# mrottmann/DDalphaAMG

Hardware: AMD Instinct MI355X
Metric: fine_wilson_clover_gflops (higher is better)
Workload: dtype f32; 1 GPU; fine Wilson-Clover apply (d_plus_clover), 32x32x32x32 local lattice per GPU, random SU(3) gauge, csw=1.0, anti-periodic T; parallelism=single, ranks=1

## Files before the change

### ddalphaamg_amd/api.py

```python
import ctypes, os, re
import numpy as np

_HERE = os.path.dirname(os.path.abspath(__file__))
_LIBNAME = os.environ.get("DDAMG_HIP_LIBRARY") or os.path.join(_HERE, "libddamg_hip.so")
_HEADER = os.path.join(os.path.dirname(_HERE), "include", "ddamg_hip.h")
MAX_LEVELS = 4
MAX_FORCE_PAIRS = 32
FORCE_GROUP = 8


class DDAMGError(RuntimeError):
    pass


class Params(ctypes.Structure):
    _fields_ = [
        ("num_levels", ctypes.c_int),
        ("local_lattice", (ctypes.c_int * 4) * MAX_LEVELS),
        ("block_lattice", (ctypes.c_int * 4) * MAX_LEVELS),
        ("num_vect", ctypes.c_int * MAX_LEVELS),
        ("post_smooth_iter", ctypes.c_int * MAX_LEVELS),
        ("block_iter", ctypes.c_int * MAX_LEVELS),
        ("setup_iter", ctypes.c_int * MAX_LEVELS),
        ("restart", ctypes.c_int), ("max_restart", ctypes.c_int),
# ... 157 lines not shown
        "ddamg_hip_force_bilinear_multi_vec": [vp, dp, ctypes.c_int, ctypes.POINTER(vp), ctypes.POINTER(vp), dp, ctypes.c_double, ctypes.c_int],
        "ddamg_hip_force_bilinear_multi_device": [vp, dp, ctypes.c_int, ctypes.POINTER(dp), ctypes.POINTER(dp), dp, ctypes.c_double, ctypes.c_int],
        "ddamg_hip_force_bilinear_multi_vec_grid": [vp, dp, ctypes.c_int, ctypes.POINTER(vp), ctypes.POINTER(vp), dp, ctypes.c_double, ctypes.c_int],
        "ddamg_hip_force_bilinear_multi_device_grid": [vp, dp, ctypes.c_int, ctypes.POINTER(dp), ctypes.POINTER(dp), dp, ctypes.c_double, ctypes.c_int],
        "ddamg_hip_force_rational_device": [vp, dp, ctypes.c_int, dp, ctypes.POINTER(dp), ctypes.POINTER(dp), ctypes.c_double, ctypes.c_int],
        "ddamg_hip_force_rational_device_grid": [vp, dp, ctypes.c_int, dp, ctypes.POINTER(dp), ctypes.POINTER(dp), ctypes.c_double, ctypes.c_int],
        "ddamg_hip_preconditioner": [vp, dp, dp],
        "ddamg_hip_residual_history": [vp, dp, ctypes.c_int, ctypes.POINTER(ctypes.c_int)],
        "ddamg_hip_get_site_order": [vp, ctypes.c_int, ctypes.POINTER(ctypes.c_int)],
        "ddamg_hip_rccl_unique_id": [vp],
        "ddamg_hip_comm_init_rccl": [vp, vp],
        "ddamg_hip_comm_init_host": [vp, EXCHANGE_FN, ALLREDUCE_FN, vp],
        "ddamg_hip_halo_plan": [ctypes.POINTER(ctypes.c_int)] * 3 + [ctypes.c_int] + [ctypes.POINTER(ctypes.c_int)] * 3,
        "ddamg_hip_timer_begin": [vp],
        "ddamg_hip_timer_end": [vp, ctypes.POINTER(ctypes.c_float)],
        "ddamg_hip_sync": [vp],
        "ddamg_hip_link_reals": [vp, ctypes.POINTER(ctypes.c_int)],
        "ddamg_hip_memory_in_use": [ctypes.POINTER(ctypes.c_size_t), ctypes.POINTER(ctypes.c_size_t)],
    }
    for name, args in sigs.items():
        fn = getattr(lib, name)
        fn.argtypes = args
        fn.restype = ctypes.c_int
    _lib = lib
    return lib


def memory_in_use():
    dev = ctypes.c_size_t(0); pin = ctypes.c_size_t(0)
    load_library().ddamg_hip_memory_in_use(ctypes.byref(dev), ctypes.byref(pin))
    return dev.value, pin.value


class VectorHeader(ctypes.Structure):
    _fields_ = [("vector_type", ctypes.c_char_p), ("m0", ctypes.c_double), ("csw", ctypes.c_double), ("clov_plaq", ctypes.c_double),
                ("hopp_plaq", ctypes.c_double), ("clov_conf_name", ctypes.c_char_p), ("hopp_conf_name", ctypes.c_char_p),
                ("has_eigenvalues", ctypes.c_int), ("eigenvalues", ctypes.POINTER(ctypes.c_double))]


class LimeInfo(ctypes.Structure):
    _fields_ = [("kind", ctypes.c_int), ("precision", ctypes.c_int), ("lattice", ctypes.c_int * 4), ("has_plaquette", ctypes.c_int),
                ("plaquette", ctypes.c_double), ("data_offset", ctypes.c_longlong), ("data_length", ctypes.c_longlong),
                ("num_records", ctypes.c_int)]


def _io():
    lib = load_library()
    if not getattr(lib, "_io_ready", False):
# ... 330 lines not shown
        cl = np.ascontiguousarray(clover_lex, dtype=np.float64)
        V = self.volume(0)
        if D.size != V * 72 or cl.size != V * 84:
            raise DDAMGError("set_operator: D must be [V][36] complex and clover [V][42] complex")
        _check(self._lib.ddamg_hip_set_operator(self._h, _dp(D), _dp(cl)))

    def shift_mass(self, m0):
        _check(self._lib.ddamg_hip_shift_mass(self._h, float(m0)))

    def scale_clover(self, scale_even, scale_odd):
        _check(self._lib.ddamg_hip_scale_clover(self._h, float(scale_even), float(scale_odd)))

    def get_operator(self):
        V = self.volume(0)
        D = np.empty((V, 36, 2)); cl = np.empty((V, 42, 2))
        _check(self._lib.ddamg_hip_get_operator(self._h, _dp(D), _dp(cl)))
        return D, cl

    def link_reals(self):
        n = ctypes.c_int(0)
        _check(self._lib.ddamg_hip_link_reals(self._h, ctypes.byref(n)))
        return n.value

    def vector(self, level=0, precision=32):
        return Vector(self, level, precision)

    def dirac_apply(self, out, inp):
        _check(self._lib.ddamg_hip_dirac_apply(self._h, out._h, inp._h))

    def dirac_apply_dagger(self, out, inp):
        _check(self._lib.ddamg_hip_dirac_apply_dagger(self._h, out._h, inp._h))

    def gamma5(self, out, inp):
        _check(self._lib.ddamg_hip_gamma5(self._h, out._h, inp._h))

    def vec_copy(self, dst, src):
        _check(self._lib.ddamg_hip_vec_copy(self._h, dst._h, src._h))

    def vec_axpy(self, z, x, y, alpha):
        alpha = complex(alpha)
        _check(self._lib.ddamg_hip_vec_axpy(self._h, z._h, x._h, y._h, alpha.real, alpha.imag))

    def vec_dot(self, x, y):
        re = ctypes.c_double(0); im = ctypes.c_double(0); nx = ctypes.c_double(0)
        _check(self._lib.ddamg_hip_vec_dot(self._h, x._h, y._h, ctypes.byref(re), ctypes.byref(im), ctypes.byref(nx)))
        return complex(re.value, im.value), nx.value
# ... 465 lines not shown
```

### ddalphaamg_amd/csrc/capi.cpp

```cpp
#include "capi_common.h"
#include "gauge.h"
#include "storage_refusal.h"
#include "ildg_device.h"
#include "io_common.h"
#include <algorithm>
#include <cmath>
#include <cstring>
#include <functional>
#include <string>
#include <fcntl.h>

using namespace ddamg;

thread_local std::string g_ddamg_last_error;

ddamg_hip_ctx::~ddamg_hip_ctx() {
  (void)hipSetDevice(device);
  if (stream) (void)hipStreamSynchronize(stream);
  mg32.reset(); mg64.reset();
  if (comm) comm_destroy(comm);
}

double* ddamg_hip_ctx::stage(size_t bytes) {
  if (bytes > d_stage.bytes()) d_stage.alloc(bytes / sizeof(double));
// ... 128 lines not shown
  *out = c.release();
  DDAMG_API_END
}

int ddamg_hip_destroy(ddamg_hip_ctx* c) {
  DDAMG_API_BEGIN
  delete c;
  DDAMG_API_END
}

int ddamg_hip_memory_in_use(size_t* device_bytes, size_t* pinned_bytes) {
  if (device_bytes) *device_bytes = DeviceMemory::in_use.load();
  if (pinned_bytes) *pinned_bytes = PinnedMemory::in_use.load();
  return 0;
}

int ddamg_hip_link_reals(ddamg_hip_ctx* c, int* reals) {
  DDAMG_API_BEGIN
  enter(c);
  DDAMG_REQUIRE(reals, "null argument");
  DDAMG_REQUIRE(c->have_operator, "link_reals: no operator uploaded");
  *reals = c->fop32.link_reals();
  DDAMG_API_END
}

int ddamg_hip_set_coarse_storage(ddamg_hip_ctx* c, int bits) { return set_storage(c, Coarse, bits, "coarse"); }
int ddamg_hip_set_transfer_storage(ddamg_hip_ctx* c, int bits) { return set_storage(c, Transfer, bits, "transfer"); }
int ddamg_hip_set_intermediate_storage(ddamg_hip_ctx* c, int bits) { return set_storage(c, Intermediate, bits, "intermediate"); }

static void drop_clover_base(ddamg_hip_ctx* c) {
  if (c->clover_base) { (void)hipStreamSynchronize(c->stream); c->clover_base.reset(); }
  c->scale_even = c->scale_odd = 1.0;
}

static void rebuild_coarse_operators(ddamg_hip_ctx* c) {
  if (c->setup_done) for_each_mg(c, [](auto& mg) { mg.operator_changed(); mg.release_setup_workspace(); });
}

static void operator_replaced(ddamg_hip_ctx* c) {
  c->have_operator = true;
  rebuild_coarse_operators(c);
}

static void upload_operator(ddamg_hip_ctx* c) {
  drop_clover_base(c);
  const Geometry& g = c->levels[0]->geom;
// ... 916 lines not shown
```

### ddalphaamg_amd/csrc/common.h

```cpp
#pragma once
#include <hip/hip_runtime.h>
#include <cstdio>
#include <cstdlib>
#include <cstdint>
#include <stdexcept>
#include <string>
#include "knobs.h"

#define DDAMG_HIP_CHECK(expr)                                                                  \
  do {                                                                                         \
    hipError_t _e = (expr);                                                                    \
    if (_e != hipSuccess) {                                                                    \
      char _buf[512];                                                                          \
      snprintf(_buf, sizeof _buf, "HIP error %s at %s:%d: %s", hipGetErrorName(_e), __FILE__,  \
               __LINE__, hipGetErrorString(_e));                                               \
      throw std::runtime_error(_buf);                                                          \
    }                                                                                          \
  } while (0)

#define DDAMG_REQUIRE(cond, msg)                                                               \
  do {                                                                                         \
    if (!(cond)) {                                                                             \
      char _buf[512];                                                                          \
      snprintf(_buf, sizeof _buf, "ddamg: requirement failed (%s) at %s:%d: %s", #cond,        \
// ... 106 lines not shown
  constexpr int NF = NR / CH;
  typedef float f4 __attribute__((ext_vector_type(4)));
  typedef double d2 __attribute__((ext_vector_type(2)));
  typedef float f2 __attribute__((ext_vector_type(2)));
#pragma unroll
  for (int k = 0; k < NF; k++) {
    auto raw = __builtin_amdgcn_raw_buffer_load_b128(b.rsrc, (int)voff, (int)(base + k * b.row), AUX);
    if constexpr (CH == 4) {
      f4 v = __builtin_bit_cast(f4, raw);
      out[4 * k] = v.x; out[4 * k + 1] = v.y; out[4 * k + 2] = v.z; out[4 * k + 3] = v.w;
    } else {
      d2 v = __builtin_bit_cast(d2, raw);
      out[2 * k] = v.x; out[2 * k + 1] = v.y;
    }
  }
  constexpr int TL = NR % CH;
  if constexpr (TL == 2) {
    f2 v = __builtin_bit_cast(f2, __builtin_amdgcn_raw_buffer_load_b64(b.rsrc, (int)(voff >> 1), (int)(base + NF * b.row), 0));
    out[NF * CH] = v.x; out[NF * CH + 1] = v.y;
  } else {
    static_assert(TL == 0, "unsupported tail width");
  }
}
#endif

template <typename T> inline size_t soa_index(int NR, size_t V, size_t s, int r) {
  constexpr int CH = Chunk<T>::CH;
  int NF = NR / CH;
  if (r < NF * CH) return ((size_t)(r / CH) * V + s) * CH + (r % CH);
  int TL = NR % CH;
  return (size_t)NF * V * CH + s * TL + (r - NF * CH);
}

}
```

### ddalphaamg_amd/csrc/fine_op.h

```cpp
#pragma once
#include "common.h"
#include "geometry.h"
#include "halo.h"

namespace ddamg {

template <typename T>
struct FineOpDev {
  const T* D;
  const T* clover;
  const T* clover_inv;
  const int* nb;
  int V;
  const T* halo;
  HaloDev hd;
  const int* tile_nb;
  const unsigned short* tnb;
  const unsigned char* parity;
  const T* Dc;
  const signed char* Dsgn;
  const T* cloverc;
  const T* Dp;
  const signed char* Dpb;
};

enum class LinkForm { Full, TwoRow, Pivot };

template <typename T>
class FineOp {
 public:
  FineOp() = default;

  void upload(const Geometry& g, const double* D_ref, const double* clover_ref, const Knobs& knobs, hipStream_t st);
  void upload_staged(const Geometry& g, const double* dD, const double* dC, const Knobs& knobs, hipStream_t st);
  void init_halo(const Geometry& g);
  void export_lex(double* dD_lex, double* dC_lex, const double* clover64, hipStream_t st) const;
  void shift_diagonal(const double* clover64, double diff, hipStream_t st);
  const T* clover_field() const { return clover_; }
  void scale_clover(const double* base64, double scale_even, double scale_odd, hipStream_t st);
  void apply(T* eta, const T* phi, hipStream_t st) const;
  void apply_dagger(T* eta, const T* phi, hipStream_t st) const;
  FineOpDev<T> dev() const { return FineOpDev<T>{D_, clover_, clover_inv_, nb_, V_, halo_.recv(), halo_.dev(), tile_nb_, tnb_, parity_, Dc_, Dsgn_, Cc_, Dp_, Dpb_}; }
  bool links_compressed() const { return Dc_ != nullptr; }
  int link_reals() const { return Dp_ ? 10 : Dc_ ? 12 : 18; }
  int V() const { return V_; }
  void apply_f32in(T* eta, const float* phi, hipStream_t st) const;
  void set_comm(Comm* c) { comm_ = c; }
  void halo_exchange(const T* v, hipStream_t st) const;
  void halo_begin(const T* v, hipStream_t st) const;
  void halo_finish(hipStream_t st) const;
  bool distributed() const { return halo_.active(); }
  void hop(T* out, const T* in, int par, hipStream_t st, int post = 0, const T* a = nullptr) const;
  void oo_inv(T* out, const T* in, hipStream_t st) const;
  void parity_select(T* out, const T* a, const T* b, int keep, hipStream_t st) const;

 private:
  template <bool DAG>
  void apply_impl(T* eta, const T* phi, hipStream_t st) const;
  void ensure_storage(const Geometry& g, hipStream_t st);
  void layout_staged(const Geometry& g, const double* dD, const double* dC, const Knobs& knobs, hipStream_t st);
  DeviceBuffer<T> D_, clover_, clover_inv_;
  DeviceBuffer<int> nb_;
  DeviceBuffer<int> lex_;
  DeviceBuffer<unsigned char> parity_;
  DeviceBuffer<int> tile_nb_;
  T* Dc_ = nullptr;
  DeviceBuffer<T> Dc_store_;
// ... 39 lines not shown
      const T pr = p == 0 ? c[0] : p == 1 ? c[2] : c[4], pi = p == 0 ? c[1] : p == 1 ? c[3] : c[5];
      const T nr = c[6] * ar + c[7] * ai + (c[8] * br + c[9] * bi);
      const T ni = c[7] * ar - c[6] * ai + (c[9] * br - c[8] * bi);
      const T inv = (T)1 / (pr * pr + pi * pi);
      const T xr = -(nr * pr - ni * pi) * inv, xi = -(nr * pi + ni * pr) * inv;
#pragma unroll
      for (int k = 0; k < 6; k++) r[k] = c[k];
      r[6] = p == 0 ? xr : c[6];                  r[7] = p == 0 ? xi : c[7];
      r[8] = p == 0 ? c[6] : p == 1 ? xr : c[8];  r[9] = p == 0 ? c[7] : p == 1 ? xi : c[9];
      r[10] = p == 2 ? xr : c[8];                 r[11] = p == 2 ? xi : c[9];
    }
#pragma unroll
    for (int k = 0; k < 12; k++) U[k] = r[k];
#pragma unroll
    for (int k = 0; k < 3; k++) {
      const int k1 = (k + 1) % 3, k2 = (k + 2) % 3;
      const T cr = r[2 * k1] * r[6 + 2 * k2] - r[2 * k1 + 1] * r[6 + 2 * k2 + 1] - (r[2 * k2] * r[6 + 2 * k1] - r[2 * k2 + 1] * r[6 + 2 * k1 + 1]);
      const T ci = r[2 * k1] * r[6 + 2 * k2 + 1] + r[2 * k1 + 1] * r[6 + 2 * k2] - (r[2 * k2] * r[6 + 2 * k1 + 1] + r[2 * k2 + 1] * r[6 + 2 * k1]);
      U[12 + 2 * k] = sg * cr; U[12 + 2 * k + 1] = -sg * ci;
    }
  }
}

template <typename T, int MU>
__device__ __forceinline__ void halo_forward(const FineOpDev<T>& op, int slot, const T (&U)[18], T (&eta)[24]) {
  T h[12], g[12];
  load_site<T, 12>(op.halo + op.hd.off[MU], (size_t)op.hd.F[MU], (size_t)slot, h);
  su3_mul<T>(U, h, g);
  spin_reconstruct_sub<T, MU, -1>(g, eta);
}
template <typename T, int MU>
__device__ __forceinline__ void halo_backward(const FineOpDev<T>& op, int slot, T (&eta)[24]) {
  T g[12];
  load_site<T, 12>(op.halo + op.hd.off[4 + MU], (size_t)op.hd.F[MU], (size_t)slot, g);
  spin_reconstruct_sub<T, MU, +1>(g, eta);
}

#endif

template <typename T>
void vec_from_lex(T* dst, const double* src_lex_dev, const int* lex_of_site, int V, int ndof, hipStream_t st, bool gamma5 = false);
template <typename T>
void vec_to_lex(double* dst_lex_dev, const T* src, const int* lex_of_site, int V, int ndof, hipStream_t st, bool gamma5 = false);

template <typename T>
void aos_from_lex(T* dst, const double* src_lex_dev, const int* lex_of_site, int V, int ndof, hipStream_t st);
template <typename T>
void aos_to_lex(double* dst_lex_dev, const T* src, const int* lex_of_site, int V, int ndof, hipStream_t st);

}
```

### ddalphaamg_amd/csrc/fine_op.hip

```cpp
#include "fine_op.h"
#include "dirac_device.h"
#include <vector>
#include <complex>
#include <cstring>

#ifndef DDAMG_NT_CLOVER
#define DDAMG_NT_CLOVER true
#endif
#ifndef DDAMG_NT_STORE
#define DDAMG_NT_STORE true
#endif
namespace ddamg {

template <bool ARITH>
__device__ __forceinline__ int tile_neighbor(const int* __restrict__ nb, size_t V, size_t s, int d, int tile0, const uint4& q,
                                             const int* __restrict__ tile_nb, int ntiles_all) {
  if constexpr (!ARITH) {
    return nb[(size_t)d * V + s];
  } else {
    const unsigned w = (d >> 1) == 0 ? q.x : (d >> 1) == 1 ? q.y : (d >> 1) == 2 ? q.z : q.w;
    const unsigned e = (d & 1) ? (w >> 16) : (w & 0xffffu);
    const int li = (int)(e & 0x7fffu);
    if (!(e & 0x8000u)) return tile0 + li;
    const int tn = tile_nb[(size_t)d * ntiles_all + (tile0 >> 8)];
// ... 12 lines not shown
    return tn >= 0 ? tn * 256 + li : nb[(size_t)d * V + s];
  }
}

template <typename T, typename TIN, int NR>
__device__ __forceinline__ void load_site_as(const TIN* __restrict__ base, size_t V, size_t s, T (&out)[NR]) {
  if constexpr (sizeof(T) == sizeof(TIN)) load_site<T, NR>(reinterpret_cast<const T*>(base), V, s, out);
  else {
    TIN tmp[NR];
    load_site<TIN, NR>(base, V, s, tmp);
#pragma unroll
    for (int k = 0; k < NR; k++) out[k] = (T)tmp[k];
  }
}

template <bool DAG, typename T>
__device__ __forceinline__ void gamma5_sign(T (&v)[24]) {
  if constexpr (DAG) {
#pragma unroll
    for (int k = 0; k < 12; k++) v[k] = -v[k];
  }
}

template <typename T, int MU, bool ARITH, LinkForm LF, bool HB2, typename TIN = T, bool CCL = false, bool DAG = false>
__device__ __forceinline__ void tile_dir(const TIN* __restrict__ phi, const FineOpDev<T>& op, size_t s, bool live, int tile0, const uint4& q,
                                         const int (&tn)[8], const T (&p)[24], T (&e)[24], T* __restrict__ sp, T* __restrict__ hb) {
  const size_t V = op.V;
  const int t = threadIdx.x;
  T U[18];
  if (live) load_link<T, MU, LF>(op, V, s, U);
  {
    T h[12], g[12];
    spin_project<T, MU, +1>(p, h);
    su3_mul_dag<T>(U, h, g);
#pragma unroll
    for (int c = 0; c < 12; c++) hb[c * 256 + t] = g[c];
  }
  if (live) {
    const int j = tile_neighbor<ARITH>(op.nb, V, s, MU, tile0, q, tn[MU]);
    if (j >= 0) {
      T pn[24];
      if (j - tile0 >= 0 && j - tile0 < 256) {
#pragma unroll
        for (int c = 0; c < 24; c++) pn[c] = sp[c * 256 + (j - tile0)];
      } else {
        load_site_as<T, TIN, 24>(phi, V, j, pn);
        gamma5_sign<DAG>(pn);
      }
      hop_accumulate<T, MU, true>(U, pn, e);
    } else {
      halo_forward<T, MU>(op, -1 - j, U, e);
    }
  }
  __syncthreads();
  if (live) {
    const int j = tile_neighbor<ARITH>(op.nb, V, s, 4 + MU, tile0, q, tn[4 + MU]);
    if (j < 0) {
      halo_backward<T, MU>(op, -1 - j, e);
    } else if (j - tile0 >= 0 && j - tile0 < 256) {
      T g[12];
#pragma unroll
      for (int c = 0; c < 12; c++) g[c] = hb[c * 256 + (j - tile0)];
      spin_reconstruct_sub<T, MU, +1>(g, e);
    } else {
      T pn[24], Un[18];
      load_site_as<T, TIN, 24>(phi, V, j, pn);
      gamma5_sign<DAG>(pn);
      load_link<T, MU, LF>(op, V, (size_t)j, Un);
      hop_accumulate<T, MU, false>(Un, pn, e);
    }
  }
  if constexpr (!HB2) __syncthreads();
}

constexpr int kDirOrder[4] = {3, 2, 0, 1};

template <typename T, bool ARITH, LinkForm LF = LinkForm::Full, typename TIN = T, bool CCL = false, bool DAG = false>
__global__ __launch_bounds__(256, (sizeof(T) == 4 ? 3 : 2)) void dirac_apply_lds_kernel(T* __restrict__ eta, const TIN* __restrict__ phi, FineOpDev<T> op, int ntiles,
                                                                  const int* __restrict__ tile_list) {
  constexpr bool HB2 = sizeof(T) == 4;
  __shared__ T sp[24 * 256];
  __shared__ T hb[(HB2 ? 2 : 1) * 12 * 256];
  T* const hb1 = hb + (HB2 ? 12 * 256 : 0);
  int tile = blockIdx.x;
  if ((ntiles & 7) == 0) tile = (blockIdx.x & 7) * (ntiles >> 3) + (blockIdx.x >> 3);
  if (tile_list) tile = tile_list[tile];
  const size_t V = op.V;
  const int tile0 = tile * 256;
  const size_t s = (size_t)tile0 + threadIdx.x;
  const bool live = s < V;
  T p[24], e[24];
  uint4 q = make_uint4(0, 0, 0, 0);
  if constexpr (ARITH) q = reinterpret_cast<const uint4*>(op.tnb)[threadIdx.x];
  int tn[8] = {0, 0, 0, 0, 0, 0, 0, 0};
  if constexpr (ARITH) {
#pragma unroll
    for (int d = 0; d < 8; d++) tn[d] = op.tile_nb[(size_t)d * (V >> 8) + tile];
  }
  if (live) {
    load_site_as<T, TIN, 24>(phi, V, s, p);
    gamma5_sign<DAG>(p);
  } else {
#pragma unroll
    for (int k = 0; k < 24; k++) p[k] = 0;
  }
#pragma unroll
  for (int c = 0; c < 24; c++) sp[c * 256 + threadIdx.x] = p[c];
  if (live) {
    if constexpr (CCL) {
      T cl[28];
      load_site<T, 28, DDAMG_NT_CLOVER>(op.cloverc, V, s, cl);
      herm6c_mul<T>(cl, p, e);
      load_site<T, 28, DDAMG_NT_CLOVER>(op.cloverc + (size_t)28 * V, V, s, cl);
      herm6c_mul<T>(cl, p + 12, e + 12);
    } else {
      T cl[36];
      load_site<T, 36, DDAMG_NT_CLOVER>(op.clover, V, s, cl);
      herm6_mul<T>(cl, p, e);
      load_site<T, 36, DDAMG_NT_CLOVER>(op.clover + (size_t)36 * V, V, s, cl);
      herm6_mul<T>(cl, p + 12, e + 12);
    }
  }
  __syncthreads();
  tile_dir<T, kDirOrder[0], ARITH, LF, HB2, TIN, CCL, DAG>(phi, op, s, live, tile0, q, tn, p, e, sp, hb);
  tile_dir<T, kDirOrder[1], ARITH, LF, HB2, TIN, CCL, DAG>(phi, op, s, live, tile0, q, tn, p, e, sp, hb1);
  tile_dir<T, kDirOrder[2], ARITH, LF, HB2, TIN, CCL, DAG>(phi, op, s, live, tile0, q, tn, p, e, sp, hb);
  tile_dir<T, kDirOrder[3], ARITH, LF, HB2, TIN, CCL, DAG>(phi, op, s, live, tile0, q, tn, p, e, sp, hb1);
  if (live) {
    gamma5_sign<DAG>(e);
    store_site<T, 24, DDAMG_NT_STORE>(eta, V, s, e);
  }
}

template <typename T, int MU, bool ARITH>
__device__ __forceinline__ void tile_dir_parity(const T* __restrict__ phi, const FineOpDev<T>& op, size_t s, bool live, bool is_out, int tile0, const uint4& q,
                                                const T (&p)[24], T (&e)[24], T* __restrict__ sp, T* __restrict__ hb) {
  const size_t V = op.V;
  const int t = threadIdx.x;
  T U[18];
  if (live) load_site<T, 18>(op.D + (size_t)MU * 18 * V, V, s, U);
  if (live && !is_out) {
    T h[12], g[12];
    spin_project<T, MU, +1>(p, h);
    su3_mul_dag<T>(U, h, g);
#pragma unroll
    for (int c = 0; c < 12; c++) hb[c * 256 + t] = g[c];
  }
  if (live && is_out) {
    const int j = tile_neighbor<ARITH>(op.nb, V, s, MU, tile0, q, op.tile_nb, (int)(V >> 8));
    if (j >= 0) {
      T pn[24];
      if (j - tile0 >= 0 && j - tile0 < 256) {
#pragma unroll
// ... 59 lines not shown
    if (post == 1) {
      T f[24], cl[36];
      load_site<T, 36>(op.clover_inv, V, s, cl);
      herm6_mul<T>(cl, e, f);
      load_site<T, 36>(op.clover_inv + (size_t)36 * V, V, s, cl);
      herm6_mul<T>(cl, e + 12, f + 12);
      store_site<T, 24>(eta, V, s, f);
    } else if (post == 2) {
      T pa[24], f[24], cl[36];
      load_site<T, 24>(a, V, s, pa);
      load_site<T, 36>(op.clover, V, s, cl);
      herm6_mul<T>(cl, pa, f);
      load_site<T, 36>(op.clover + (size_t)36 * V, V, s, cl);
      herm6_mul<T>(cl, pa + 12, f + 12);
#pragma unroll
      for (int k = 0; k < 24; k++) f[k] -= e[k];
      store_site<T, 24>(eta, V, s, f);
    } else {
      store_site<T, 24>(eta, V, s, e);
    }
  }
}

template <typename T, bool CCL, bool DAG>
static void launch_dirac_apply(T* eta, const T* phi, const FineOpDev<T>& op, int ntiles, const int* tile_list, hipStream_t st) {
  if constexpr (sizeof(T) == 4) {
    if (op.tnb && op.Dp) {
      hipLaunchKernelGGL((dirac_apply_lds_kernel<T, true, LinkForm::Pivot, T, CCL, DAG>), dim3(ntiles), dim3(256), 0, st, eta, phi, op, ntiles, tile_list);
      return;
    }
  }
  if (op.tnb && op.Dc) hipLaunchKernelGGL((dirac_apply_lds_kernel<T, true, LinkForm::TwoRow, T, CCL, DAG>), dim3(ntiles), dim3(256), 0, st, eta, phi, op, ntiles, tile_list);
  else if (op.tnb) hipLaunchKernelGGL((dirac_apply_lds_kernel<T, true, LinkForm::Full, T, CCL, DAG>), dim3(ntiles), dim3(256), 0, st, eta, phi, op, ntiles, tile_list);
  else hipLaunchKernelGGL((dirac_apply_lds_kernel<T, false, LinkForm::Full, T, CCL, DAG>), dim3(ntiles), dim3(256), 0, st, eta, phi, op, ntiles, tile_list);
}

template <typename T>
template <bool DAG>
void FineOp<T>::apply_impl(T* eta, const T* phi, hipStream_t st) const {
  DDAMG_REQUIRE(D_ != nullptr, "fine operator not uploaded");
  auto launch = [&](int ntiles, const int* tile_list) {
    if (ntiles == 0) return;
    if (Cc_) launch_dirac_apply<T, sizeof(T) == 4, DAG>(eta, phi, dev(), ntiles, tile_list, st);
    else launch_dirac_apply<T, false, DAG>(eta, phi, dev(), ntiles, tile_list, st);
    DDAMG_HIP_CHECK(hipGetLastError());
  };
  if (!halo_.active()) {
    launch((V_ + 255) / 256, nullptr);
    return;
  }
  halo_.pack(phi, D_, V_, st, DAG);
  halo_.exchange_begin(comm_, st);
  launch(halo_.n_interior(), halo_.interior_tiles());
  halo_.exchange_finish(comm_, st);
  launch(halo_.n_boundary(), halo_.boundary_tiles());
}
template <typename T>
void FineOp<T>::apply(T* eta, const T* phi, hipStream_t st) const { apply_impl<false>(eta, phi, st); }
template <typename T>
void FineOp<T>::apply_dagger(T* eta, const T* phi, hipStream_t st) const {
  DDAMG_REQUIRE(eta != phi, "apply_dagger: in place");
  apply_impl<true>(eta, phi, st);
}

template <>
void FineOp<double>::apply_f32in(double* eta, const float* phi, hipStream_t st) const {
  DDAMG_REQUIRE(D_ != nullptr, "fine operator not uploaded");
  auto launch = [&](int ntiles, const int* tile_list) {
    if (ntiles == 0) return;
    if (tnb_ && Dc_) hipLaunchKernelGGL((dirac_apply_lds_kernel<double, true, LinkForm::TwoRow, float>), dim3(ntiles), dim3(256), 0, st, eta, phi, dev(), ntiles, tile_list);
    else if (tnb_) hipLaunchKernelGGL((dirac_apply_lds_kernel<double, true, LinkForm::Full, float>), dim3(ntiles), dim3(256), 0, st, eta, phi, dev(), ntiles, tile_list);
    else hipLaunchKernelGGL((dirac_apply_lds_kernel<double, false, LinkForm::Full, float>), dim3(ntiles), dim3(256), 0, st, eta, phi, dev(), ntiles, tile_list);
    DDAMG_HIP_CHECK(hipGetLastError());
  };
  if (!halo_.active()) { launch((V_ + 255) / 256, nullptr); return; }
  halo_.pack_f32in(phi, D_, V_, st);
  halo_.exchange_begin(comm_, st);
  launch(halo_.n_interior(), halo_.interior_tiles());
  halo_.exchange_finish(comm_, st);
  launch(halo_.n_boundary(), halo_.boundary_tiles());
}

template <typename T>
void FineOp<T>::hop(T* eta, const T* phi, int par, hipStream_t st, int post, const T* a) const {
  DDAMG_REQUIRE(post == 0 || post == 1 || (post == 2 && a != nullptr && a != eta), "hop: unknown epilogue");
  DDAMG_REQUIRE(D_ != nullptr, "fine operator not uploaded");
  auto launch = [&](int ntiles, const int* tile_list) {
    if (ntiles == 0) return;
    if (tnb_) hipLaunchKernelGGL((dirac_hop_parity_kernel<T, true>), dim3(ntiles), dim3(256), 0, st, eta, phi, dev(), ntiles, tile_list, par, post, a);
    else hipLaunchKernelGGL((dirac_hop_parity_kernel<T, false>), dim3(ntiles), dim3(256), 0, st, eta, phi, dev(), ntiles, tile_list, par, post, a);
    DDAMG_HIP_CHECK(hipGetLastError());
  };
  if (!halo_.active()) { launch((V_ + 255) / 256, nullptr); return; }
  halo_.pack(phi, D_, V_, st);
  halo_.exchange_begin(comm_, st);
// ... 581 lines not shown
```

### include/ddamg_hip.h

```cpp
#ifndef DDAMG_HIP_H
#define DDAMG_HIP_H

#include <stddef.h>

#ifdef __cplusplus
extern "C" {
#endif

#define DDAMG_HIP_MAX_LEVELS 4

typedef struct ddamg_hip_ctx ddamg_hip_ctx;
typedef struct ddamg_hip_vec ddamg_hip_vec;
typedef struct ddamg_hip_chrono ddamg_hip_chrono;

typedef struct ddamg_hip_params {
  int num_levels;
  int local_lattice[DDAMG_HIP_MAX_LEVELS][4];
  int block_lattice[DDAMG_HIP_MAX_LEVELS][4];
  int num_vect[DDAMG_HIP_MAX_LEVELS];
  int post_smooth_iter[DDAMG_HIP_MAX_LEVELS];
  int block_iter[DDAMG_HIP_MAX_LEVELS];
  int setup_iter[DDAMG_HIP_MAX_LEVELS];
  int restart, max_restart;
  double tol;
// ... 168 lines not shown
                                    const double* const* x_o_dev, double coeff, int accumulate);
int ddamg_hip_force_rational_device_grid(ddamg_hip_ctx* ctx, double* force_dev, int nshift, const double* rho, const double* const* x_e_dev,
                                         const double* const* x_o_dev, double coeff, int accumulate);

int ddamg_hip_residual_history(ddamg_hip_ctx* ctx, double* history, int max_len, int* len);

int ddamg_hip_get_site_order(ddamg_hip_ctx* ctx, int level, int* lex_of_site);

typedef struct ddamg_hip_halo_msg {
  int send_peer, recv_peer;
  int tag;
  const void* send;
  void* recv;
  unsigned long long bytes;
} ddamg_hip_halo_msg;
typedef void (*ddamg_hip_exchange_fn)(void* user, int nmsg, const ddamg_hip_halo_msg* msgs);
typedef void (*ddamg_hip_allreduce_fn)(void* user, double* buf, int n);
int ddamg_hip_rccl_unique_id(void* id128);
int ddamg_hip_comm_init_rccl(ddamg_hip_ctx* ctx, const void* id128);
int ddamg_hip_comm_init_host(ddamg_hip_ctx* ctx, ddamg_hip_exchange_fn fn, ddamg_hip_allreduce_fn reduce_fn, void* user);
const char* ddamg_hip_comm_stats(ddamg_hip_ctx* ctx, int reset);
int ddamg_hip_memory_in_use(size_t* device_bytes, size_t* pinned_bytes);
int ddamg_hip_link_reals(ddamg_hip_ctx* ctx, int* reals);
int ddamg_hip_halo_plan(const int local_lattice[4], const int process_grid[4], const int process_coords[4],
                        int face, int* neighbor_rank, int* count, int* lex_sites);

int ddamg_hip_timer_begin(ddamg_hip_ctx* ctx);
int ddamg_hip_timer_end(ddamg_hip_ctx* ctx, float* milliseconds);
int ddamg_hip_sync(ddamg_hip_ctx* ctx);

#ifdef __cplusplus
}
#endif
#endif
```

Measured before the change: 16930 GFLOP/s.

## Use 32-bit buffer-resource addressing in fine Dirac apply and hoist first link/clover loads

Adds an O32 variant of the fine Wilson-Clover LDS kernel that builds AMD buffer resource descriptors for phi, eta, links, clover, halo and neighbour tables, so loads and stores use 32-bit offsets instead of 64-bit pointer arithmetic. The variant is chosen at launch when every field fits in 32-bit byte offsets. It also moves the first direction's link load and the clover loads up beside the spinor load, and drops one barrier for the first direction. The aim is to cut address-calculation instructions and VGPR use and to overlap memory latency. The cost is more template instantiations and possible register-pressure changes, plus new API query functions.

```diff
diff --git a/ddalphaamg_amd/api.py b/ddalphaamg_amd/api.py
--- a/ddalphaamg_amd/api.py
+++ b/ddalphaamg_amd/api.py
@@ -203,8 +203,22 @@
         fn = getattr(lib, name)
         fn.argtypes = args
         fn.restype = ctypes.c_int
+    ull = ctypes.c_ulonglong
+    newer = {
+        "ddamg_hip_offset_bits": [vp, ctypes.c_int, ctypes.POINTER(ctypes.c_int)],
+        "ddamg_hip_field_fits_32bit": [ull, ull, ull],
+    }
+    for name, args in newer.items():
+        if hasattr(lib, name):
+            fn = getattr(lib, name)
+            fn.argtypes = args
+            fn.restype = ctypes.c_int
     _lib = lib
     return lib
+
+
+def field_fits_32bit(sites, reals_per_site, bytes_per_real):
+    return bool(load_library().ddamg_hip_field_fits_32bit(int(sites), int(reals_per_site), int(bytes_per_real)))
 
 
 def memory_in_use():
@@ -581,6 +595,11 @@
         _check(self._lib.ddamg_hip_link_reals(self._h, ctypes.byref(n)))
         return n.value
 
+    def offset_bits(self, precision=32):
+        n = ctypes.c_int(0)
+        _check(self._lib.ddamg_hip_offset_bits(self._h, int(precision), ctypes.byref(n)))
+        return n.value
+
     def vector(self, level=0, precision=32):
         return Vector(self, level, precision)
 
diff --git a/ddalphaamg_amd/csrc/capi.cpp b/ddalphaamg_amd/csrc/capi.cpp
--- a/ddalphaamg_amd/csrc/capi.cpp
+++ b/ddalphaamg_amd/csrc/capi.cpp
@@ -174,6 +174,20 @@
   DDAMG_REQUIRE(c->have_operator, "link_reals: no operator uploaded");
   *reals = c->fop32.link_reals();
   DDAMG_API_END
+}
+
+int ddamg_hip_offset_bits(ddamg_hip_ctx* c, int precision, int* bits) {
+  DDAMG_API_BEGIN
+  enter(c);
+  DDAMG_REQUIRE(bits, "null argument");
+  DDAMG_REQUIRE(precision == 32 || precision == 64, "offset_bits: precision is 32 or 64");
+  DDAMG_REQUIRE(c->have_operator, "offset_bits: no operator uploaded");
+  *bits = (precision == 32 ? c->fop32.offsets_32bit() : c->fop64.offsets_32bit()) ? 32 : 64;
+  DDAMG_API_END
+}
+
+int ddamg_hip_field_fits_32bit(unsigned long long sites, unsigned long long reals_per_site, unsigned long long bytes_per_real) {
+  return ddamg::field_fits_32bit(sites, reals_per_site, bytes_per_real) ? 1 : 0;
 }
 
 int ddamg_hip_set_coarse_storage(ddamg_hip_ctx* c, int bits) { return set_storage(c, Coarse, bits, "coarse"); }
diff --git a/ddalphaamg_amd/csrc/common.h b/ddalphaamg_amd/csrc/common.h
--- a/ddalphaamg_amd/csrc/common.h
+++ b/ddalphaamg_amd/csrc/common.h
@@ -152,7 +152,42 @@
     static_assert(TL == 0, "unsupported tail width");
   }
 }
+__device__ __forceinline__ SiteBuf make_field_buf(const void* p, size_t V, unsigned bytes) {
+  SiteBuf b;
+  b.rsrc = __builtin_amdgcn_make_buffer_rsrc(const_cast<void*>(p), 0, (int)bytes, 0x00020000);
+  b.row = (unsigned)(V * 16);
+  return b;
+}
+template <typename T, int NR, int AUX = 0>
+__device__ __forceinline__ void store_site_b(const SiteBuf& b, unsigned base, unsigned voff, const T (&in)[NR]) {
+  constexpr int CH = Chunk<T>::CH;
+  constexpr int NF = NR / CH;
+  static_assert(NR % CH == 0, "whole 16-byte chunks");
+  typedef float f4 __attribute__((ext_vector_type(4)));
+  typedef double d2 __attribute__((ext_vector_type(2)));
+#pragma unroll
+  for (int k = 0; k < NF; k++) {
+    if constexpr (CH == 4) {
+      const f4 v = {in[4 * k], in[4 * k + 1], in[4 * k + 2], in[4 * k + 3]};
+      __builtin_amdgcn_raw_buffer_store_b128(__builtin_bit_cast(decltype(__builtin_amdgcn_raw_buffer_load_b128(b.rsrc, 0, 0, 0)), v), b.rsrc, (int)voff, (int)(base + k * b.row), AUX);
+    } else {
+      const d2 v = {in[2 * k], in[2 * k + 1]};
+      __builtin_amdgcn_raw_buffer_store_b128(__builtin_bit_cast(decltype(__builtin_amdgcn_raw_buffer_load_b128(b.rsrc, 0, 0, 0)), v), b.rsrc, (int)voff, (int)(base + k * b.row), AUX);
+    }
+  }
+}
+__device__ __forceinline__ int load_byte_b(const SiteBuf& b, unsigned base, unsigned site) {
+  return (int)(signed char)__builtin_amdgcn_raw_buffer_load_b8(b.rsrc, (int)site, (int)base, 0);
+}
 #endif
+
+inline bool field_fits_32bit(unsigned long long V, unsigned long long reals, unsigned long long elem_bytes) {
+  const unsigned long long lim = 1ull << 32;
+  if (V == 0 || reals == 0 || elem_bytes == 0) return true;
+  if (V >= lim || reals >= lim || elem_bytes >= lim) return false;
+  const unsigned long long per_site = reals * elem_bytes;
+  return per_site < lim && V <= (lim - 1) / per_site;
+}
 
 template <typename T> inline size_t soa_index(int NR, size_t V, size_t s, int r) {
   constexpr int CH = Chunk<T>::CH;
diff --git a/ddalphaamg_amd/csrc/fine_op.h b/ddalphaamg_amd/csrc/fine_op.h
--- a/ddalphaamg_amd/csrc/fine_op.h
+++ b/ddalphaamg_amd/csrc/fine_op.h
@@ -43,6 +43,7 @@
   FineOpDev<T> dev() const { return FineOpDev<T>{D_, clover_, clover_inv_, nb_, V_, halo_.recv(), halo_.dev(), tile_nb_, tnb_, parity_, Dc_, Dsgn_, Cc_, Dp_, Dpb_}; }
   bool links_compressed() const { return Dc_ != nullptr; }
   int link_reals() const { return Dp_ ? 10 : Dc_ ? 12 : 18; }
+  bool offsets_32bit() const;
   int V() const { return V_; }
   void apply_f32in(T* eta, const float* phi, hipStream_t st) const;
   void set_comm(Comm* c) { comm_ = c; }
@@ -128,6 +129,47 @@
   }
 }
 
+template <typename T, int MU, LinkForm LF>
+__device__ __forceinline__ void load_link_b(const SiteBuf& links, const SiteBuf& bytes, unsigned V, unsigned voff, T (&U)[18]) {
+  if constexpr (LF == LinkForm::Full) {
+    load_site_b<T, 18>(links, (unsigned)MU * 18u * (unsigned)sizeof(T) * V, voff, U);
+  } else {
+    T r[12];
+    T sg;
+    if constexpr (LF == LinkForm::TwoRow) {
+      load_site_b<T, 12>(links, (unsigned)MU * 12u * (unsigned)sizeof(T) * V, voff, r);
+      sg = (T)2 * (T)load_byte_b(bytes, (unsigned)MU * V, voff >> 4);
+    } else {
+      T c[10];
+      load_site_b<T, 10>(links, (unsigned)MU * 10u * (unsigned)sizeof(T) * V, voff, c);
+      const int b = load_byte_b(bytes, (unsigned)MU * V, voff >> 4);
+      sg = b < 0 ? (T)-2 : (T)2;
+      const int p = (b < 0 ? -b : b) - 1;
+      const T ar = p == 0 ? c[2] : c[0], ai = p == 0 ? c[3] : c[1];
+      const T br = p == 2 ? c[2] : c[4], bi = p == 2 ? c[3] : c[5];
+      const T pr = p == 0 ? c[0] : p == 1 ? c[2] : c[4], pi = p == 0 ? c[1] : p == 1 ? c[3] : c[5];
+      const T nr = c[6] * ar + c[7] * ai + (c[8] * br + c[9] * bi);
+      const T ni = c[7] * ar - c[6] * ai + (c[9] * br - c[8] * bi);
+      const T inv = (T)1 / (pr * pr + pi * pi);
+      const T xr = -(nr * pr - ni * pi) * inv, xi = -(nr * pi + ni * pr) * inv;
+#pragma unroll
+      for (int k = 0; k < 6; k++) r[k] = c[k];
+      r[6] = p == 0 ? xr : c[6];                  r[7] = p == 0 ? xi : c[7];
+      r[8] = p == 0 ? c[6] : p == 1 ? xr : c[8];  r[9] = p == 0 ? c[7] : p == 1 ? xi : c[9];
+      r[10] = p == 2 ? xr : c[8];                 r[11] = p == 2 ? xi : c[9];
+    }
+#pragma unroll
+    for (int k = 0; k < 12; k++) U[k] = r[k];
+#pragma unroll
+    for (int k = 0; k < 3; k++) {
+      const int k1 = (k + 1) % 3, k2 = (k + 2) % 3;
+      const T cr = r[2 * k1] * r[6 + 2 * k2] - r[2 * k1 + 1] * r[6 + 2 * k2 + 1] - (r[2 * k2] * r[6 + 2 * k1] - r[2 * k2 + 1] * r[6 + 2 * k1 + 1]);
+      const T ci = r[2 * k1] * r[6 + 2 * k2 + 1] + r[2 * k1 + 1] * r[6 + 2 * k2] - (r[2 * k2] * r[6 + 2 * k1 + 1] + r[2 * k2 + 1] * r[6 + 2 * k1]);
+      U[12 + 2 * k] = sg * cr; U[12 + 2 * k + 1] = -sg * ci;
+    }
+  }
+}
+
 template <typename T, int MU>
 __device__ __forceinline__ void halo_forward(const FineOpDev<T>& op, int slot, const T (&U)[18], T (&eta)[24]) {
   T h[12], g[12];
@@ -142,6 +184,22 @@
   spin_reconstruct_sub<T, MU, +1>(g, eta);
 }
 
+template <typename T, int MU>
+__device__ __forceinline__ void halo_forward_b(const SiteBuf& halo, const HaloDev& hd, int slot, const T (&U)[18], T (&eta)[24]) {
+  T h[12], g[12];
+  SiteBuf hb = halo; hb.row = (unsigned)hd.F[MU] * 16u;
+  load_site_b<T, 12>(hb, (unsigned)hd.off[MU] * (unsigned)sizeof(T), (unsigned)slot * 16u, h);
+  su3_mul<T>(U, h, g);
+  spin_reconstruct_sub<T, MU, -1>(g, eta);
+}
+template <typename T, int MU>
+__device__ __forceinline__ void halo_backward_b(const SiteBuf& halo, const HaloDev& hd, int slot, T (&eta)[24]) {
+  T g[12];
+  SiteBuf hb = halo; hb.row = (unsigned)hd.F[MU] * 16u;
+  load_site_b<T, 12>(hb, (unsigned)hd.off[4 + MU] * (unsigned)sizeof(T), (unsigned)slot * 16u, g);
+  spin_reconstruct_sub<T, MU, +1>(g, eta);
+}
+
 #endif
 
 template <typename T>
diff --git a/ddalphaamg_amd/csrc/fine_op.hip b/ddalphaamg_amd/csrc/fine_op.hip
--- a/ddalphaamg_amd/csrc/fine_op.hip
+++ b/ddalphaamg_amd/csrc/fine_op.hip
@@ -58,41 +58,99 @@
   }
 }
 
-template <typename T, int MU, bool ARITH, LinkForm LF, bool HB2, typename TIN = T, bool CCL = false, bool DAG = false>
-__device__ __forceinline__ void tile_dir(const TIN* __restrict__ phi, const FineOpDev<T>& op, size_t s, bool live, int tile0, const uint4& q,
-                                         const int (&tn)[8], const T (&p)[24], T (&e)[24], T* __restrict__ sp, T* __restrict__ hb) {
+template <bool O32> struct ApplyBufs {};
+template <> struct ApplyBufs<true> {
+  SiteBuf phi, eta;
+  SiteBuf links, lbytes;
+  SiteBuf clover;
+  SiteBuf halo;
+  SiteBuf nb;
+};
+template <typename T, typename TIN, LinkForm LF, bool CCL>
+__device__ __forceinline__ ApplyBufs<true> make_apply_bufs(T* eta, const TIN* phi, const FineOpDev<T>& op) {
+  const unsigned V = (unsigned)op.V;
+  ApplyBufs<true> bf;
+  bf.phi = make_field_buf(phi, V, 24u * (unsigned)sizeof(TIN) * V);
+  bf.eta = make_field_buf(eta, V, 24u * (unsigned)sizeof(T) * V);
+  if constexpr (LF == LinkForm::Full) { bf.links = make_field_buf(op.D, V, 72u * (unsigned)sizeof(T) * V); bf.lbytes = bf.links; }
+  else if constexpr (LF == LinkForm::TwoRow) { bf.links = make_field_buf(op.Dc, V, 48u * (unsigned)sizeof(T) * V); bf.lbytes = make_field_buf(op.Dsgn, V, 4u * V); }
+  else { bf.links = make_field_buf(op.Dp, V, 40u * (unsigned)sizeof(T) * V); bf.lbytes = make_field_buf(op.Dpb, V, 4u * V); }
+  if constexpr (CCL) bf.clover = make_field_buf(op.cloverc, V, 56u * (unsigned)sizeof(T) * V);
+  else bf.clover = make_field_buf(op.clover, V, 72u * (unsigned)sizeof(T) * V);
+  bf.halo = make_field_buf(op.halo, V, 24u * (unsigned)sizeof(T) * (unsigned)(op.hd.F[0] + op.hd.F[1] + op.hd.F[2] + op.hd.F[3]));
+  bf.nb = make_field_buf(op.nb, V, 32u * V);
+  return bf;
+}
+template <typename T, typename TIN, bool O32>
+__device__ __forceinline__ void apply_load_phi(const TIN* __restrict__ phi, const ApplyBufs<O32>& bf, size_t V, size_t s, T (&out)[24]) {
+  if constexpr (!O32) load_site_as<T, TIN, 24>(phi, V, s, out);
+  else if constexpr (sizeof(T) == sizeof(TIN)) load_site_b<T, 24>(bf.phi, 0u, (unsigned)s * 16u, out);
+  else {
+    TIN tmp[24];
+    load_site_b<TIN, 24>(bf.phi, 0u, (unsigned)s * 16u, tmp);
+#pragma unroll
+    for (int k = 0; k < 24; k++) out[k] = (T)tmp[k];
+  }
+}
+template <bool ARITH, bool O32>
+__device__ __forceinline__ int apply_neighbor(const int* __restrict__ nb, const ApplyBufs<O32>& bf, size_t V, size_t s, int d, int tile0, const uint4& q, int tn) {
+  if constexpr (!O32) return tile_neighbor<ARITH>(nb, V, s, d, tile0, q, tn);
+  else {
+    const unsigned base = (unsigned)d * 4u * (unsigned)V, voff = (unsigned)s * 4u;
+    if constexpr (!ARITH) {
+      return (int)__builtin_amdgcn_raw_buffer_load_b32(bf.nb.rsrc, (int)voff, (int)base, 0);
+    } else {
+      const unsigned w = (d >> 1) == 0 ? q.x : (d >> 1) == 1 ? q.y : (d >> 1) == 2 ? q.z : q.w;
+      const unsigned e = (d & 1) ? (w >> 16) : (w & 0xffffu);
+      const int li = (int)(e & 0x7fffu);
+      if (!(e & 0x8000u)) return tile0 + li;
+      return tn >= 0 ? tn * 256 + li : (int)__builtin_amdgcn_raw_buffer_load_b32(bf.nb.rsrc, (int)voff, (int)base, 0);
+    }
+  }
+}
+template <typename T, int MU, LinkForm LF, bool O32>
+__device__ __forceinline__ void apply_load_link(const FineOpDev<T>& op, const ApplyBufs<O32>& bf, size_t V, size_t s, T (&U)[18]) {
+  if constexpr (O32) load_link_b<T, MU, LF>(bf.links, bf.lbytes, (unsigned)V, (unsigned)s * 16u, U);
+  else load_link<T, MU, LF>(op, V, s, U);
+}
+
+template <typename T, int MU>
+__device__ __forceinline__ void tile_dir_products(const T (&U)[18], const T (&p)[24], T* __restrict__ hb) {
+  T h[12], g[12];
+  spin_project<T, MU, +1>(p, h);
+  su3_mul_dag<T>(U, h, g);
+#pragma unroll
+  for (int c = 0; c < 12; c++) hb[c * 256 + threadIdx.x] = g[c];
+}
+
+template <typename T, int MU, bool ARITH, LinkForm LF, bool HB2, bool BAR, typename TIN, bool CCL, bool DAG, bool O32>
+__device__ __forceinline__ void tile_dir_terms(const TIN* __restrict__ phi, const FineOpDev<T>& op, const ApplyBufs<O32>& bf, size_t s, bool live, int tile0,
+                                               const uint4& q, const int (&tn)[8], const T (&U)[18], T (&e)[24], const T* __restrict__ sp,
+                                               const T* __restrict__ hb) {
   const size_t V = op.V;
-  const int t = threadIdx.x;
-  T U[18];
-  if (live) load_link<T, MU, LF>(op, V, s, U);
-  {
-    T h[12], g[12];
-    spin_project<T, MU, +1>(p, h);
-    su3_mul_dag<T>(U, h, g);
-#pragma unroll
-    for (int c = 0; c < 12; c++) hb[c * 256 + t] = g[c];
-  }
   if (live) {
-    const int j = tile_neighbor<ARITH>(op.nb, V, s, MU, tile0, q, tn[MU]);
+    const int j = apply_neighbor<ARITH, O32>(op.nb, bf, V, s, MU, tile0, q, tn[MU]);
     if (j >= 0) {
       T pn[24];
       if (j - tile0 >= 0 && j - tile0 < 256) {
 #pragma unroll
         for (int c = 0; c < 24; c++) pn[c] = sp[c * 256 + (j - tile0)];
       } else {
-        load_site_as<T, TIN, 24>(phi, V, j, pn);
+        apply_load_phi<T, TIN, O32>(phi, bf, V, (size_t)j, pn);
         gamma5_sign<DAG>(pn);
       }
       hop_accumulate<T, MU, true>(U, pn, e);
     } else {
-      halo_forward<T, MU>(op, -1 - j, U, e);
-    }
-  }
-  __syncthreads();
+      if constexpr (O32) halo_forward_b<T, MU>(bf.halo, op.hd, -1 - j, U, e);
+      else halo_forward<T, MU>(op, -1 - j, U, e);
+    }
+  }
+  if constexpr (BAR) __syncthreads();
   if (live) {
-    const int j = tile_neighbor<ARITH>(op.nb, V, s, 4 + MU, tile0, q, tn[4 + MU]);
+    const int j = apply_neighbor<ARITH, O32>(op.nb, bf, V, s, 4 + MU, tile0, q, tn[4 + MU]);
     if (j < 0) {
-      halo_backward<T, MU>(op, -1 - j, e);
+      if constexpr (O32) halo_backward_b<T, MU>(bf.halo, op.hd, -1 - j, e);
+      else halo_backward<T, MU>(op, -1 - j, e);
     } else if (j - tile0 >= 0 && j - tile0 < 256) {
       T g[12];
 #pragma unroll
@@ -100,18 +158,26 @@
       spin_reconstruct_sub<T, MU, +1>(g, e);
     } else {
       T pn[24], Un[18];
-      load_site_as<T, TIN, 24>(phi, V, j, pn);
+      apply_load_phi<T, TIN, O32>(phi, bf, V, (size_t)j, pn);
       gamma5_sign<DAG>(pn);
-      load_link<T, MU, LF>(op, V, (size_t)j, Un);
+      apply_load_link<T, MU, LF, O32>(op, bf, V, (size_t)j, Un);
       hop_accumulate<T, MU, false>(Un, pn, e);
     }
   }
   if constexpr (!HB2) __syncthreads();
 }
+template <typename T, int MU, bool ARITH, LinkForm LF, bool HB2, typename TIN, bool CCL, bool DAG, bool O32>
+__device__ __forceinline__ void tile_dir(const TIN* __restrict__ phi, const FineOpDev<T>& op, const ApplyBufs<O32>& bf, size_t s, bool live, int tile0,
+                                         const uint4& q, const int (&tn)[8], const T (&p)[24], T (&e)[24], T* __restrict__ sp, T* __restrict__ hb) {
+  T U[18];
+  if (live) apply_load_link<T, MU, LF, O32>(op, bf, op.V, s, U);
+  tile_dir_products<T, MU>(U, p, hb);
+  tile_dir_terms<T, MU, ARITH, LF, HB2, true, TIN, CCL, DAG, O32>(phi, op, bf, s, live, tile0, q, tn, U, e, sp, hb);
+}
 
 constexpr int kDirOrder[4] = {3, 2, 0, 1};
 
-template <typename T, bool ARITH, LinkForm LF = LinkForm::Full, typename TIN = T, bool CCL = false, bool DAG = false>
+template <typename T, bool ARITH, LinkForm LF = LinkForm::Full, typename TIN = T, bool CCL = false, bool DAG = false, bool O32 = false>
 __global__ __launch_bounds__(256, (sizeof(T) == 4 ? 3 : 2)) void dirac_apply_lds_kernel(T* __restrict__ eta, const TIN* __restrict__ phi, FineOpDev<T> op, int ntiles,
                                                                   const int* __restrict__ tile_list) {
   constexpr bool HB2 = sizeof(T) == 4;
@@ -125,7 +191,9 @@
   const int tile0 = tile * 256;
   const size_t s = (size_t)tile0 + threadIdx.x;
   const bool live = s < V;
-  T p[24], e[24];
+  ApplyBufs<O32> bf;
+  if constexpr (O32) bf = make_apply_bufs<T, TIN, LF, CCL>(eta, phi, op);
+  T p[24], e[24], U0[18];
   uint4 q = make_uint4(0, 0, 0, 0);
   if constexpr (ARITH) q = reinterpret_cast<const uint4*>(op.tnb)[threadIdx.x];
   int tn[8] = {0, 0, 0, 0, 0, 0, 0, 0};
@@ -133,8 +201,13 @@
 #pragma unroll
     for (int d = 0; d < 8; d++) tn[d] = op.tile_nb[(size_t)d * (V >> 8) + tile];
   }
+  constexpr int NCL = CCL ? 28 : 36;
+  T cl[NCL];
   if (live) {
-    load_site_as<T, TIN, 24>(phi, V, s, p);
+    apply_load_phi<T, TIN, O32>(phi, bf, V, s, p);
+    apply_load_link<T, kDirOrder[0], LF, O32>(op, bf, V, s, U0);
+    if constexpr (O32) load_site_b<T, NCL, DDAMG_NT_CLOVER ? 2 : 0>(bf.clover, 0u, (unsigned)s * 16u, cl);
+    else load_site<T, NCL, DDAMG_NT_CLOVER>(CCL ? op.cloverc : op.clover, V, s, cl);
     gamma5_sign<DAG>(p);
   } else {
 #pragma unroll
@@ -142,29 +215,29 @@
   }
 #pragma unroll
   for (int c = 0; c < 24; c++) sp[c * 256 + threadIdx.x] = p[c];
+  tile_dir_products<T, kDirOrder[0]>(U0, p, hb);
   if (live) {
     if constexpr (CCL) {
-      T cl[28];
-      load_site<T, 28, DDAMG_NT_CLOVER>(op.cloverc, V, s, cl);
       herm6c_mul<T>(cl, p, e);
-      load_site<T, 28, DDAMG_NT_CLOVER>(op.cloverc + (size_t)28 * V, V, s, cl);
+      if constexpr (O32) load_site_b<T, 28, DDAMG_NT_CLOVER ? 2 : 0>(bf.clover, 28u * (unsigned)sizeof(T) * (unsigned)V, (unsigned)s * 16u, cl);
+      else load_site<T, 28, DDAMG_NT_CLOVER>(op.cloverc + (size_t)28 * V, V, s, cl);
       herm6c_mul<T>(cl, p + 12, e + 12);
     } else {
-      T cl[36];
-      load_site<T, 36, DDAMG_NT_CLOVER>(op.clover, V, s, cl);
       herm6_mul<T>(cl, p, e);
-      load_site<T, 36, DDAMG_NT_CLOVER>(op.clover + (size_t)36 * V, V, s, cl);
+      if constexpr (O32) load_site_b<T, 36, DDAMG_NT_CLOVER ? 2 : 0>(bf.clover, 36u * (unsigned)sizeof(T) * (unsigned)V, (unsigned)s * 16u, cl);
+      else load_site<T, 36, DDAMG_NT_CLOVER>(op.clover + (size_t)36 * V, V, s, cl);
       herm6_mul<T>(cl, p + 12, e + 12);
     }
   }
   __syncthreads();
-  tile_dir<T, kDirOrder[0], ARITH, LF, HB2, TIN, CCL, DAG>(phi, op, s, live, tile0, q, tn, p, e, sp, hb);
-  tile_dir<T, kDirOrder[1], ARITH, LF, HB2, TIN, CCL, DAG>(phi, op, s, live, tile0, q, tn, p, e, sp, hb1);
-  tile_dir<T, kDirOrder[2], ARITH, LF, HB2, TIN, CCL, DAG>(phi, op, s, live, tile0, q, tn, p, e, sp, hb);
-  tile_dir<T, kDirOrder[3], ARITH, LF, HB2, TIN, CCL, DAG>(phi, op, s, live, tile0, q, tn, p, e, sp, hb1);
+  tile_dir_terms<T, kDirOrder[0], ARITH, LF, HB2, false, TIN, CCL, DAG, O32>(phi, op, bf, s, live, tile0, q, tn, U0, e, sp, hb);
+  tile_dir<T, kDirOrder[1], ARITH, LF, HB2, TIN, CCL, DAG, O32>(phi, op, bf, s, live, tile0, q, tn, p, e, sp, hb1);
+  tile_dir<T, kDirOrder[2], ARITH, LF, HB2, TIN, CCL, DAG, O32>(phi, op, bf, s, live, tile0, q, tn, p, e, sp, hb);
+  tile_dir<T, kDirOrder[3], ARITH, LF, HB2, TIN, CCL, DAG, O32>(phi, op, bf, s, live, tile0, q, tn, p, e, sp, hb1);
   if (live) {
     gamma5_sign<DAG>(e);
-    store_site<T, 24, DDAMG_NT_STORE>(eta, V, s, e);
+    if constexpr (O32) store_site_b<T, 24, DDAMG_NT_STORE ? 2 : 0>(bf.eta, 0u, (unsigned)s * 16u, e);
+    else store_site<T, 24, DDAMG_NT_STORE>(eta, V, s, e);
   }
 }
 
@@ -270,17 +343,30 @@
   }
 }
 
-template <typename T, bool CCL, bool DAG>
-static void launch_dirac_apply(T* eta, const T* phi, const FineOpDev<T>& op, int ntiles, const int* tile_list, hipStream_t st) {
+template <typename T, typename TIN, bool CCL, bool DAG, bool O32>
+static void launch_dirac_apply_form(T* eta, const TIN* phi, const FineOpDev<T>& op, int ntiles, const int* tile_list, hipStream_t st) {
   if constexpr (sizeof(T) == 4) {
     if (op.tnb && op.Dp) {
-      hipLaunchKernelGGL((dirac_apply_lds_kernel<T, true, LinkForm::Pivot, T, CCL, DAG>), dim3(ntiles), dim3(256), 0, st, eta, phi, op, ntiles, tile_list);
+      hipLaunchKernelGGL((dirac_apply_lds_kernel<T, true, LinkForm::Pivot, TIN, CCL, DAG, O32>), dim3(ntiles), dim3(256), 0, st, eta, phi, op, ntiles, tile_list);
       return;
     }
   }
-  if (op.tnb && op.Dc) hipLaunchKernelGGL((dirac_apply_lds_kernel<T, true, LinkForm::TwoRow, T, CCL, DAG>), dim3(ntiles), dim3(256), 0, st, eta, phi, op, ntiles, tile_list);
-  else if (op.tnb) hipLaunchKernelGGL((dirac_apply_lds_kernel<T, true, LinkForm::Full, T, CCL, DAG>), dim3(ntiles), dim3(256), 0, st, eta, phi, op, ntiles, tile_list);
-  else hipLaunchKernelGGL((dirac_apply_lds_kernel<T, false, LinkForm::Full, T, CCL, DAG>), dim3(ntiles), dim3(256), 0, st, eta, phi, op, ntiles, tile_list);
+  if (op.tnb && op.Dc) hipLaunchKernelGGL((dirac_apply_lds_kernel<T, true, LinkForm::TwoRow, TIN, CCL, DAG, O32>), dim3(ntiles), dim3(256), 0, st, eta, phi, op, ntiles, tile_list);
+  else if (op.tnb) hipLaunchKernelGGL((dirac_apply_lds_kernel<T, true, LinkForm::Full, TIN, CCL, DAG, O32>), dim3(ntiles), dim3(256), 0, st, eta, phi, op, ntiles, tile_list);
+  else hipLaunchKernelGGL((dirac_apply_lds_kernel<T, false, LinkForm::Full, TIN, CCL, DAG, O32>), dim3(ntiles), dim3(256), 0, st, eta, phi, op, ntiles, tile_list);
+}
+template <typename T, typename TIN, bool CCL, bool DAG>
+static void launch_dirac_apply(T* eta, const TIN* phi, const FineOpDev<T>& op, bool o32, int ntiles, const int* tile_list, hipStream_t st) {
+  if (o32) launch_dirac_apply_form<T, TIN, CCL, DAG, true>(eta, phi, op, ntiles, tile_list, st);
+  else launch_dirac_apply_form<T, TIN, CCL, DAG, false>(eta, phi, op, ntiles, tile_list, st);
+}
+
+template <typename T>
+bool FineOp<T>::offsets_32bit() const {
+  const int link = (sizeof(T) == 4 && tnb_ && Dp_) ? 40 : (tnb_ && Dc_) ? 48 : 72;
+  const int clov = (sizeof(T) == 4 && Cc_) ? 56 : 72;
+  const unsigned long long V = (unsigned long long)V_;
+  return field_fits_32bit(V, 24, sizeof(T)) && field_fits_32bit(V, (unsigned long long)link, sizeof(T)) && field_fits_32bit(V, (unsigned long long)clov, sizeof(T));
 }
 
 template <typename T>
@@ -289,8 +375,8 @@
   DDAMG_REQUIRE(D_ != nullptr, "fine operator not uploaded");
   auto launch = [&](int ntiles, const int* tile_list) {
     if (ntiles == 0) return;
-    if (Cc_) launch_dirac_apply<T, sizeof(T) == 4, DAG>(eta, phi, dev(), ntiles, tile_list, st);
-    else launch_dirac_apply<T, false, DAG>(eta, phi, dev(), ntiles, tile_list, st);
+    if (Cc_) launch_dirac_apply<T, T, sizeof(T) == 4, DAG>(eta, phi, dev(), offsets_32bit(), ntiles, tile_list, st);
+    else launch_dirac_apply<T, T, false, DAG>(eta, phi, dev(), offsets_32bit(), ntiles, tile_list, st);
     DDAMG_HIP_CHECK(hipGetLastError());
   };
   if (!halo_.active()) {
@@ -316,9 +402,7 @@
   DDAMG_REQUIRE(D_ != nullptr, "fine operator not uploaded");
   auto launch = [&](int ntiles, const int* tile_list) {
     if (ntiles == 0) return;
-    if (tnb_ && Dc_) hipLaunchKernelGGL((dirac_apply_lds_kernel<double, true, LinkForm::TwoRow, float>), dim3(ntiles), dim3(256), 0, st, eta, phi, dev(), ntiles, tile_list);
-    else if (tnb_) hipLaunchKernelGGL((dirac_apply_lds_kernel<double, true, LinkForm::Full, float>), dim3(ntiles), dim3(256), 0, st, eta, phi, dev(), ntiles, tile_list);
-    else hipLaunchKernelGGL((dirac_apply_lds_kernel<double, false, LinkForm::Full, float>), dim3(ntiles), dim3(256), 0, st, eta, phi, dev(), ntiles, tile_list);
+    launch_dirac_apply<double, float, false, false>(eta, phi, dev(), offsets_32bit(), ntiles, tile_list, st);
     DDAMG_HIP_CHECK(hipGetLastError());
   };
   if (!halo_.active()) { launch((V_ + 255) / 256, nullptr); return; }
diff --git a/include/ddamg_hip.h b/include/ddamg_hip.h
--- a/include/ddamg_hip.h
+++ b/include/ddamg_hip.h
@@ -214,6 +214,8 @@
 const char* ddamg_hip_comm_stats(ddamg_hip_ctx* ctx, int reset);
 int ddamg_hip_memory_in_use(size_t* device_bytes, size_t* pinned_bytes);
 int ddamg_hip_link_reals(ddamg_hip_ctx* ctx, int* reals);
+int ddamg_hip_offset_bits(ddamg_hip_ctx* ctx, int precision, int* bits);
+int ddamg_hip_field_fits_32bit(unsigned long long sites, unsigned long long reals_per_site, unsigned long long bytes_per_real);
 int ddamg_hip_halo_plan(const int local_lattice[4], const int process_grid[4], const int process_coords[4],
                         int face, int* neighbor_rank, int* count, int* lex_sites);
 
```

Result: no change. 16860 GFLOP/s (-0.4%).
